# jchristopherson/nonlin

Hardware: AMD Instinct MI355X
Metric: LM iterations/sec on m=4096,n=256 fp64; FD-Jacobian GB/s vs HBM peak (higher is better)
Workload: dtype f64

## Files before the change

include/nonlin_hip.h:

```cpp
#ifndef NONLIN_HIP_H
#define NONLIN_HIP_H

#include <stdint.h>

#ifdef __cplusplus
extern "C" {
#endif

#define NLH_NO_ERROR                     0
#define NLH_INVALID_INPUT_ERROR        201
#define NLH_ARRAY_SIZE_ERROR           202
#define NLH_OUT_OF_MEMORY_ERROR        105
#define NLH_INVALID_OPERATION_ERROR    104
#define NLH_CONVERGENCE_ERROR          106
#define NLH_DIVERGENT_BEHAVIOR_ERROR   206
#define NLH_SPURIOUS_CONVERGENCE_ERROR 207
#define NLH_TOLERANCE_TOO_SMALL_ERROR  208
#define NLH_DIVIDE_BY_ZERO_ERROR       210
#define NLH_UNDEFINED_FUNCTION_ERROR   211
#define NLH_UNDERDEFINED_PROBLEM_ERROR 212
#define NLH_ERR_NO_DEVICE             -1
#define NLH_ERR_HIP                   -2
#define NLH_ERR_BAD_HANDLE            -3

// ... 654 lines not shown
                            nlh_iteration_behavior *ib, int32_t *status);
int nlh_curve_fit_batch_sep_h(nlh_handle *h, const nlh_options *opts, int32_t kind, int32_t ncomp, int32_t nbase, int32_t nprob,
                              int32_t m, const double *t, int32_t shared_t, const double *y, const double *w, int32_t analytic,
                              const double *xl, const double *xu, const nlh_group *g, const nlh_conv *cv, const nlh_sep *sp,
                              double *x, double *fvec, double *sigma, double *cov, double *chi2, int32_t *rank,
                              nlh_iteration_behavior *ib, int32_t *status);
int nlh_expr_fit_batch_sep(nlh_handle *h, const nlh_options *opts, const nlh_expr *e, int32_t nprob, int32_t m, const double *dt,
                           int32_t shared_t, const double *dy, const double *dw, int32_t analytic, const double *xl,
                           const double *xu, const nlh_group *g, const nlh_conv *cv, const nlh_sep *sp, double *dx, double *dfvec,
                           double *dsigma, double *dcov, double *dchi2, int32_t *drank, nlh_iteration_behavior *ib,
                           int32_t *status);
int nlh_expr_fit_batch_sep_h(nlh_handle *h, const nlh_options *opts, const nlh_expr *e, int32_t nprob, int32_t m, const double *t,
                             int32_t shared_t, const double *y, const double *w, int32_t analytic, const double *xl,
                             const double *xu, const nlh_group *g, const nlh_conv *cv, const nlh_sep *sp, double *x, double *fvec,
                             double *sigma, double *cov, double *chi2, int32_t *rank, nlh_iteration_behavior *ib,
                             int32_t *status);

#define NLH_K_DQ_RESIDUAL   0
#define NLH_K_DQ_PANEL      1
#define NLH_K_FD_JACOBIAN   2
#define NLH_K_GRAM          3
#define NLH_K_GRAM_REDUCE   4
#define NLH_K_JTF           5
#define NLH_K_CHOL          6
#define NLH_K_LMPAR         7
#define NLH_K_QR            8
#define NLH_K_UPDATE        9
#define NLH_K_LU           10
#define NLH_K_DQ_JACOBIAN  11
#define NLH_K_QRX_PASS     12
#define NLH_K_QRX_PIVOT    13
#define NLH_K_POLYROOTS    14
#define NLH_K_COVAR       15
#define NLH_K_COUNT        16
void nlh_timing_enable(nlh_handle *h, int32_t on);
void nlh_timing_reset(nlh_handle *h);
int  nlh_timing_get(nlh_handle *h, int32_t kernel_id, double *total_ms, int64_t *launches);
int64_t nlh_timing_samples(nlh_handle *h, int32_t kernel_id, float *out_ms, int64_t cap);
const char *nlh_kernel_name(int32_t kernel_id);

#ifdef __cplusplus
}
#endif

#include "nonlin_hip_guess.h"

#include "nonlin_hip_starts.h"

#include "nonlin_hip_boot.h"

#include "nonlin_hip_bin.h"

#include "nonlin_hip_boot_pois.h"

#endif
```

nonlin_amd/_lib.py:

```python
import ctypes as C
import math
import os

_HERE = os.path.dirname(os.path.abspath(__file__))
LIB_PATH = os.path.join(_HERE, "libnonlin_hip.so")

c_double_p = C.POINTER(C.c_double)
c_int32_p = C.POINTER(C.c_int32)

VECFCN = C.CFUNCTYPE(None, C.c_void_p, C.c_int32, c_double_p, C.c_int32, c_double_p)
JACFCN = C.CFUNCTYPE(None, C.c_void_p, C.c_int32, c_double_p, C.c_int32, c_double_p)
FCNNVAR = C.CFUNCTYPE(C.c_double, C.c_void_p, C.c_int32, c_double_p)
GRADFCN = C.CFUNCTYPE(None, C.c_void_p, C.c_int32, c_double_p, c_double_p)
DEVFCN = C.CFUNCTYPE(C.c_int, C.c_void_p, C.c_void_p, C.c_int32, C.c_void_p, C.c_int32, C.c_void_p, C.c_int32, C.c_void_p)


class IterationBehavior(C.Structure):
    _fields_ = [(k, C.c_int32) for k in (
        "iter_count", "fcn_count", "jacobian_count", "gradient_count",
        "converge_on_fcn", "converge_on_chng", "converge_on_zero_diff")]

    def as_dict(self):
        return {k: int(getattr(self, k)) for k, _ in self._fields_}

# ... 318 lines not shown
                                        C.c_void_p, C.c_int32, C.c_void_p, C.c_void_p]),
    "nlh_curve_guess_batch_h": (C.c_int, [_H, C.c_int32, C.c_int32, C.c_int32, C.c_int32, C.c_int32, c_double_p, C.c_int32, c_double_p,
                                          c_double_p, C.c_int32, c_double_p, c_int32_p]),
}

_STARTS_BOX = [c_double_p, c_double_p, c_int32_p]
STARTS_SYMBOLS = {
    "nlh_starts_candidates": (C.c_int, [C.c_int32, C.c_int32, C.c_int32] + _STARTS_BOX + [c_double_p]),
    "nlh_starts_search_batch_device": (C.c_int, [_H, C.c_int32, C.c_int32, C.c_int32, DEVFCN, C.c_void_p] + _STARTS_BOX +
                                       [C.c_int32, C.c_int32, C.c_void_p, C.c_void_p, C.c_void_p]),
    "nlh_starts_search_batch_device_h": (C.c_int, [_H, C.c_int32, C.c_int32, C.c_int32, DEVFCN, C.c_void_p] + _STARTS_BOX +
                                         [C.c_int32, C.c_int32, c_double_p, c_double_p, c_int32_p]),
    "nlh_starts_cost_batch": (C.c_int, [_H, C.c_int32, C.c_int32, C.c_void_p, C.c_void_p]),
    "nlh_starts_pick_batch": (C.c_int, [_H, C.c_int32, C.c_int32, C.c_void_p, C.c_void_p]),
    "nlh_starts_take_batch": (C.c_int, [_H, C.c_int32, C.c_int32, C.c_int32, C.c_void_p, C.c_void_p, C.c_void_p]),
}

BOOT_SYMBOLS = {
    "nlh_boot_draws": (C.c_int, [C.c_uint64, C.c_int64, C.c_int32, C.c_int32, C.c_int32, C.c_int32, c_int32_p]),
    "nlh_boot_resample_batch": (C.c_int, [_H, C.c_int32, C.c_uint64, C.c_int32, C.c_int64, C.c_int32, C.c_int32, C.c_int32, C.c_void_p,
                                          C.c_void_p, C.c_void_p, C.c_int32, C.c_void_p, C.c_void_p]),
    "nlh_boot_summary_batch": (C.c_int, [_H, C.c_int32, C.c_int32, C.c_int32, C.c_void_p, C.c_double, C.c_void_p, C.c_void_p, C.c_void_p,
                                         C.c_void_p, C.c_void_p]),
}

BIN_SYMBOLS = {
    "nlh_bin_rule": (C.c_int, [C.c_int32, c_double_p, c_double_p]),
    "nlh_bin_wrap": (C.c_int, [_H, C.c_void_p, C.c_void_p, C.c_void_p, DEVFCN, DEVFCN, C.c_void_p, C.POINTER(C.c_void_p)]),
    "nlh_bin_unwrap": _RELEASE,
    "nlh_bin_device_fcn": _LAUNCHER,
    "nlh_bin_device_jac": _LAUNCHER,
    "nlh_bin_apply_batch": (C.c_int, [_H, C.c_void_p, C.c_int32, C.c_int32, C.c_int32, C.c_void_p, C.c_void_p]),
}

BOOT_POIS_SYMBOLS = {
    "nlh_boot_poisson_draws": (C.c_int, [C.c_uint64, C.c_int64, C.c_int32, C.c_int32, C.c_int32, c_double_p, c_double_p]),
    "nlh_boot_poisson_batch": (C.c_int, [_H, C.c_uint64, C.c_int32, C.c_int64, C.c_int32, C.c_int32, C.c_int32, C.c_void_p, C.c_void_p,
                                         C.c_void_p, C.c_void_p, C.c_void_p]),
}

KERNEL_IDS = {
    "dq_residual": 0, "dq_panel": 1, "fd_jacobian": 2, "gram": 3, "gram_reduce": 4, "jtf": 5,
    "chol": 6, "lmpar": 7, "qr": 8, "update": 9, "lu": 10, "dq_jacobian": 11, "qrx_pass": 12, "qrx_pivot": 13,
    "polyroots": 14, "covar": 15,
}

_lib = None


class NonlinHipUnavailable(RuntimeError):
    pass


def load():
    global _lib
    if _lib is not None:
        return _lib
    if not os.path.exists(LIB_PATH):
        raise NonlinHipUnavailable(
            f"{LIB_PATH} not found: build it with `python -c 'import __graft_entry__ as g; g.build()'` "
            "or `make -C nonlin_amd/csrc` (there is no CPU fallback)")
    try:
        import torch
    except ImportError:
        pass
    lib = C.CDLL(LIB_PATH)
    for name, (res, args) in (list(SYMBOLS.items()) + list(GUESS_SYMBOLS.items()) + list(STARTS_SYMBOLS.items()) + list(BOOT_SYMBOLS.items()) +
                              list(BIN_SYMBOLS.items()) + list(BOOT_POIS_SYMBOLS.items())):
        fn = getattr(lib, name)
        fn.restype = res
        fn.argtypes = args
    _lib = lib
    return lib


def default_options():
    o = Options()
    load().nlh_default_options(C.byref(o))
    return o


CURVE_GAUSS, CURVE_LORENTZ, CURVE_EXPDECAY = 0, 1, 2
CURVE_KINDS = {"gauss": CURVE_GAUSS, "lorentz": CURVE_LORENTZ, "expdecay": CURVE_EXPDECAY}


def curve_kind(kind):
    if isinstance(kind, str):
        if kind not in CURVE_KINDS:
            raise ValueError(f"unknown curve kind {kind!r}: one of {sorted(CURVE_KINDS)}")
        return CURVE_KINDS[kind]
    return int(kind)


def curve_nparams(kind, ncomp=1, baseline=-1):
    n = load().nlh_curve_nparams(curve_kind(kind), int(ncomp), int(baseline))
    if n < 0:
        raise ValueError(f"no curve model of kind {kind!r} with {ncomp} components and baseline degree {baseline}")
    return n


GUESS_FALLBACK, GUESS_RANKDEF, GUESS_NONE = 1, 2, 4
GUESS_MAX_M = 8192


EXPR_OPS = ("CONST", "VAR", "PARAM", "NEG", "ADD", "SUB", "MUL", "DIV", "IPOW", "POWC", "EXP", "LOG", "SQRT", "SIN", "COS", "TANH",
            "ATAN", "ABS")
EXPR_SPECIAL_OPS = ("ERF", "ERFC", "ERFCX", "VOIGT")
EXPR_EXTENDED_OPS = ("POW", "ATAN2", "MIN", "MAX", "WHERE")
EXPR_DEF_OPS = ("LOAD",)
EXPR_SPECIAL2_OPS = ("J0", "J1", "I0E", "I1E", "LGAMMA", "EXPM1", "LOG1P")


def faddeeva_table():
    import numpy as np
    L, a = C.c_double(), np.zeros(40)
    load().nlh_faddeeva_table(C.byref(L), a.ctypes.data_as(c_double_p))
    return L.value, a


def wofz(z):
    import numpy as np
# ... 623 lines not shown
```

nonlin_amd/csrc/nlh_core.hip:

```cpp
#include "nlh_internal.h"
#include "nlh_kernels_model.h"
#include "nlh_qrx.h"

int ensure(nlh_handle *h, DevBuf &b, size_t bytes)
{
    if (bytes <= b.bytes && b.p) return 0;
    if (b.p) { hipFree(b.p); b.p = nullptr; b.bytes = 0; }
    size_t want = bytes < 256 ? 256 : bytes;
    hipError_t e = hipMalloc(&b.p, want);
    if (e != hipSuccess) { h->err = std::string("hipMalloc: ") + hipGetErrorString(e); return NLH_OUT_OF_MEMORY_ERROR; }
    b.bytes = want;
    bool known = false;
    for (auto *q : h->bufs) if (q == &b) known = true;
    if (!known) h->bufs.push_back(&b);
    return 0;
}

bool lds_fits(const void *kernel, size_t dyn)
{
    static std::mutex mu;
    static std::vector<std::pair<const void *, size_t>> statics;
    size_t st = 0;
    {
        std::lock_guard<std::mutex> g(mu);
        auto it = std::find_if(statics.begin(), statics.end(), [&](const std::pair<const void *, size_t> &e) { return e.first == kernel; });
        if (it != statics.end()) st = it->second;
        else {
            hipFuncAttributes a;
            if (hipFuncGetAttributes(&a, kernel) != hipSuccess) return false;
            st = a.sharedSizeBytes;
            statics.emplace_back(kernel, st);
        }
    }
    return st + dyn <= (size_t)NLH_LDS_MAX;
}

int ensure_staging(nlh_handle *h, size_t bytes)
{
    if (bytes <= h->staging_bytes) return 0;
    if (h->staging) hipHostFree(h->staging);
    h->staging = nullptr; h->staging_bytes = 0;
    if (hipHostMalloc(&h->staging, bytes, hipHostMallocDefault) != hipSuccess) { h->err = "hipHostMalloc (staging)"; return NLH_OUT_OF_MEMORY_ERROR; }
    h->staging_bytes = bytes;
    return 0;
}

int ensure_pinned(nlh_handle *h, size_t bytes)
{
    if (bytes <= h->pinned_bytes) return 0;
    if (h->pinned) hipHostFree(h->pinned);
    h->pinned = nullptr; h->pinned_bytes = 0;
    hipError_t e = hipHostMalloc(&h->pinned, bytes, hipHostMallocDefault);
    if (e != hipSuccess) { h->err = std::string("hipHostMalloc: ") + hipGetErrorString(e); return NLH_OUT_OF_MEMORY_ERROR; }
    h->pinned_bytes = bytes;
    return 0;
// ... 29 lines not shown
void nlh_default_options(nlh_options *o)
{
    o->max_evals = 100;
    o->ftol = 1.0e-8;
    o->xtol = 1.0e-12;
    o->gtol = 1.0e-12;
    o->print_status = 0;
    o->factor = 100.0;
    o->use_line_search = 1;
    o->ls_max_evals = 100;
    o->ls_alpha = 1.0e-4;
    o->ls_factor = 0.1;
    o->factor_policy = NLH_FACTOR_EXACT;
    o->ne_pivot_tol = 1.0e-4;
    o->fuse_fd = 1;
    o->sub_batches = 0;
}

int nlh_device_count(void)
{
    int n = 0;
    if (hipGetDeviceCount(&n) != hipSuccess) return 0;
    return n;
}

const char *nlh_version(void) { return "nonlin_hip 0.1 (gfx950)"; }

int nlh_create(nlh_handle **out, int32_t device, void *hip_stream)
{
    if (!out) return NLH_ERR_BAD_HANDLE;
    *out = nullptr;
    if (nlh_device_count() <= 0) return NLH_ERR_NO_DEVICE;
    if (hipSetDevice(device) != hipSuccess) return NLH_ERR_NO_DEVICE;
    nlh_handle *h = new nlh_handle();
    h->device = device;
    h->stream = (hipStream_t)hip_stream;
    const int lds_max = NLH_LDS_MAX;
    qrx_init_device();
    nlh_lm_init_device(lds_max);
    nlh_square_init_device(lds_max);
    nlh_cls_init_device(lds_max);
    nlh_bfgs_init_device(lds_max);
    nlh_poly_init_device(lds_max);
    nlh_polyroots_init_device(lds_max);
    nlh_covar_init_device(lds_max);
    nlh_devfcn_init_device(lds_max);
    nlh_expr_init_device(lds_max);
    nlh_sep_init_device(lds_max);
    nlh_band_init_device(lds_max);
    nlh_guess_init_device(lds_max);
    nlh_boot_init_device(lds_max);
    (void)hipFuncSetAttribute((const void *)k_dq_residual<RB>, hipFuncAttributeMaxDynamicSharedMemorySize, lds_max);
    (void)hipFuncSetAttribute((const void *)k_dq_residual2<RB / 2>, hipFuncAttributeMaxDynamicSharedMemorySize, lds_max);
    (void)hipGetLastError();
    *out = h;
    return 0;
}

void nlh_destroy(nlh_handle *h)
{
    if (!h) return;
    for (auto *wk : h->workers) nlh_destroy(wk);
    h->workers.clear();
    hipSetDevice(h->device);
    hipStreamSynchronize(h->stream);
    timing_flush(h);
    for (auto e : h->pool) hipEventDestroy(e);
    for (auto *b : h->bufs) if (b->p) hipFree(b->p);
    if (h->pinned) hipHostFree(h->pinned);
    if (h->staging) hipHostFree(h->staging);
    if (h->cbstage) hipHostFree(h->cbstage);
    if (h->lu_side) { hipStreamSynchronize(h->lu_side); hipStreamDestroy(h->lu_side); }
    if (h->lu_panel_done) hipEventDestroy(h->lu_panel_done);
    for (auto e : h->lu_bulk_done) if (e) hipEventDestroy(e);
    if (h->own_stream) hipStreamDestroy(h->stream);
    delete h;
}

const char *nlh_last_error(const nlh_handle *h) { return h ? h->err.c_str() : "null handle"; }

void nlh_timing_enable(nlh_handle *h, int32_t on)
{
    if (!h) return;
    h->timing = on == 0 ? 0u : on == 1 ? 0xffffffffu : ((uint32_t)on >> 1);
}
void nlh_timing_reset(nlh_handle *h)
{
    if (!h) return;
    timing_flush(h);
    for (int k = 0; k < NLH_K_COUNT; ++k) { h->ms[k] = 0; h->launches[k] = 0; }
    h->samples.clear();
}
int64_t nlh_timing_samples(nlh_handle *h, int32_t kid, float *out_ms, int64_t cap)
{
    if (!h) return NLH_ERR_BAD_HANDLE;
    if (kid != h->sample_kid) {
        timing_flush(h);
        h->sample_kid = kid;
        h->samples.clear();
        return 0;
    }
    timing_flush(h);
    const int64_t cnt = (int64_t)h->samples.size();
    for (int64_t i = 0; i < cnt && i < cap; ++i) out_ms[i] = h->samples[(size_t)i];
    return cnt;
}
// ... 28 lines not shown
    for (size_t e = (size_t)blockIdx.x * blockDim.x + threadIdx.x; e < mn + (size_t)n; e += (size_t)gridDim.x * blockDim.x) {
        const double u = 2.0 * sm64_u(seed, e) - 1.0;
        if (e < mn) {
            double v = u / rs;
            const size_t i = e % m, j = e / m;
            if (square_shift && i == j) v = 2.0 + v;
            A[(size_t)p * mn + e] = v;
        } else {
            xtrue[(size_t)p * n + (e - mn)] = u;
        }
    }
}

__global__ void k_gen_bx(int m, int n, uint64_t seed0, uint64_t stride, double sigma, double spread, double *b,
                         const double *xtrue, double *x0)
{
    const int p = blockIdx.y;
    const uint64_t seed = seed0 + (uint64_t)p * stride;
    const size_t base = (size_t)m * n + (size_t)n;
    for (size_t e = (size_t)blockIdx.x * blockDim.x + threadIdx.x; e < (size_t)m + n; e += (size_t)gridDim.x * blockDim.x) {
        const double u = 2.0 * sm64_u(seed, base + e) - 1.0;
        if (e < (size_t)m) b[(size_t)p * m + e] = b[(size_t)p * m + e] + sigma * u;
        else x0[(size_t)p * n + (e - m)] = xtrue[(size_t)p * n + (e - m)] + spread * u;
    }
}


void launch_dq_residual(nlh_handle *h, int nprob, int m, int n, const double *A, const double *b,
                               double gamma, const double *x, double *f, double *part,
                               const LmState *st, int want)
{
    Timed t(h, NLH_K_DQ_RESIDUAL);
    size_t sh = sizeof(double) * (size_t)(n + 32);
    const bool vec2 = (m % 2 == 0) && ((((uintptr_t)A | (uintptr_t)b | (uintptr_t)f) & 15) == 0);
    const int nblk = (m + RB - 1) / RB;
    lockstep_slices(nprob, [&](int32_t p0, int32_t cnt) {
        dim3 grid(nblk, cnt);
        const double *Ap = A + (size_t)p0 * m * n, *bp = b + (size_t)p0 * m, *xp = x + (size_t)p0 * n;
        double *fp = f + (size_t)p0 * m, *pp = part ? part + (size_t)p0 * nblk * 2 : nullptr;
        const LmState *sp = st ? st + p0 : nullptr;
        if (vec2)
            hipLaunchKernelGGL(k_dq_residual2<RB / 2>, grid, dim3(RB / 2), sh, h->stream, m, n, Ap, bp, gamma, xp, fp, pp, sp, want);
        else
            hipLaunchKernelGGL(k_dq_residual<RB>, grid, dim3(RB), sh, h->stream, m, n, Ap, bp, gamma, xp, fp, pp, sp, want);
        return 0;
    });
}

void launch_dq_panel(nlh_handle *h, int nprob, int m, int n, const double *A, const double *b,
                            double gamma, const double *x, double *P, const LmState *st, int want,
                            const double *f0_fused, bool to_qrx)
{
    Timed t(h, NLH_K_DQ_PANEL);
    constexpr int JT = 32;
    dim3 grid((m + RB - 1) / RB, (n + JT - 1) / JT, nprob);
    size_t sh = sizeof(double) * (size_t)n;
    const int tld = to_qrx ? qrx_ld(n) : 0, tcoff = to_qrx ? qrx_ld(n) - (n + 1) : 0;
    const size_t tst = to_qrx ? qrx_matrix_stride(m, n) : 0;
    if (f0_fused)
        hipLaunchKernelGGL((k_dq_panel<RB, JT, true>), grid, dim3(RB), sh, h->stream, m, n, A, b, gamma, x, P, f0_fused, st, want,
                           tld, tcoff, tst);
    else
        hipLaunchKernelGGL((k_dq_panel<RB, JT, false>), grid, dim3(RB), sh, h->stream, m, n, A, b, gamma, x, P,
                           (const double *)nullptr, st, want, 0, 0, (size_t)0);
}

void launch_fd(nlh_handle *h, int nprob, int m, int n, const double *P, const double *f0,
                      const double *x, double *J, const LmState *st, int want)
{
    Timed t(h, NLH_K_FD_JACOBIAN);
    constexpr int CJ = 8;
    const bool vec2 = (m % 2 == 0) && ((((uintptr_t)P | (uintptr_t)J | (uintptr_t)f0) & 15) == 0);
    if (vec2) {
        dim3 grid((m / 2 + RB - 1) / RB, (n + CJ - 1) / CJ, nprob);
        hipLaunchKernelGGL((k_fd_jacobian<RB, CJ, true>), grid, dim3(RB), 0, h->stream, m, n, P, f0, x, J, st, want);
    } else {
        dim3 grid((m + RB - 1) / RB, (n + CJ - 1) / CJ, nprob);
        hipLaunchKernelGGL((k_fd_jacobian<RB, CJ, false>), grid, dim3(RB), 0, h->stream, m, n, P, f0, x, J, st, want);
    }
}

void format_e10_3(double v, char out[16])
{
    char body[16];
    if (std::isnan(v)) { snprintf(out, 16, "%10s", "NaN"); return; }
    if (std::isinf(v)) { snprintf(out, 16, "%10s", v < 0 ? "-Inf" : "Inf"); return; }
    char sci[32];
    snprintf(sci, sizeof sci, "%.2e", fabs(v));
    int ex = atoi(sci + 5);
    if (v != 0.0) ex += 1;
    const char sign = std::signbit(v) && v != 0.0 ? '-' : ' ';
    if (abs(ex) < 100) snprintf(body, sizeof body, "%c0.%c%c%cE%c%02d", sign, sci[0], sci[2], sci[3], ex < 0 ? '-' : '+', abs(ex));
    else snprintf(body, sizeof body, "%c0.%c%c%c%c%03d", sign, sci[0], sci[2], sci[3], ex < 0 ? '-' : '+', abs(ex));
    snprintf(out, 16, "%10s", body);
}

void print_status(int iter, int nfeval, int njaceval, double xnorm, double fnorm)
{
    char a[16], b[16];
    format_e10_3(xnorm, a);
    format_e10_3(fnorm, b);
    printf(" \nIteration: %d\nFunction Evaluations: %d\n", iter, nfeval);
    if (njaceval > 0) printf("Jacobian Evaluations: %d\n", njaceval);
    printf("Change in Variable: %s\nResidual: %s\n", a, b);
    fflush(stdout);
}

int nlh_format_status(int32_t iter, int32_t nfeval, int32_t njaceval, double xnorm, double fnorm, char *buf,
                                 int32_t len)
// ... 32 lines not shown


int ensure_workers(nlh_handle *h, int T)
{
    while ((int)h->workers.size() < T) {
        nlh_handle *wk = new nlh_handle();
        wk->device = h->device;
        if (hipStreamCreateWithFlags(&wk->stream, hipStreamNonBlocking) != hipSuccess) { delete wk; h->err = "hipStreamCreate"; return NLH_ERR_HIP; }
        wk->own_stream = true;
        h->workers.push_back(wk);
    }
    return 0;
}

int nlh_dq_generate(nlh_handle *h, int32_t nprob, int32_t m, int32_t n, uint64_t seed0, uint64_t seed_stride, double gamma,
                    double sigma, double spread, int32_t square_shift, double *dA, double *db,
                    double *dxtrue, double *dx0)
{
    if (!h) return NLH_ERR_BAD_HANDLE;
    HIPCHK(h, hipSetDevice(h->device));
    const size_t mn = (size_t)m * n;
    unsigned gx = (unsigned)((mn + n + 255) / 256);
    if (gx > 4096) gx = 4096;
    hipLaunchKernelGGL(k_gen_A, dim3(gx, nprob), dim3(256), 0, h->stream, m, n, seed0, seed_stride, square_shift, dA, dxtrue);
    HIPCHK(h, hipMemsetAsync(db, 0, sizeof(double) * (size_t)nprob * m, h->stream));
    launch_dq_residual(h, nprob, m, n, dA, db, gamma, dxtrue, db, nullptr, nullptr, -1);
    unsigned gb = (unsigned)(((size_t)m + n + 255) / 256);
    hipLaunchKernelGGL(k_gen_bx, dim3(gb, nprob), dim3(256), 0, h->stream, m, n, seed0, seed_stride, sigma, spread, db, dxtrue, dx0);
    HIPCHK(h, hipGetLastError());
    return 0;
}

int nlh_dq_residual(nlh_handle *h, int32_t nprob, int32_t m, int32_t n, const double *dA, const double *db,
                    double gamma, const double *dx, double *df)
{
    if (!h) return NLH_ERR_BAD_HANDLE;
    HIPCHK(h, hipSetDevice(h->device));
    launch_dq_residual(h, nprob, m, n, dA, db, gamma, dx, df, nullptr, nullptr, -1);
    HIPCHK(h, hipGetLastError());
    return 0;
}

int nlh_dq_fd_panel(nlh_handle *h, int32_t nprob, int32_t m, int32_t n, const double *dA, const double *db,
                    double gamma, const double *dx, double *dP)
{
    if (!h) return NLH_ERR_BAD_HANDLE;
    if (m < 1 || n < 1) return NLH_INVALID_INPUT_ERROR;
    HIPCHK(h, hipSetDevice(h->device));
    launch_dq_panel(h, nprob, m, n, dA, db, gamma, dx, dP, nullptr, -1);
    HIPCHK(h, hipGetLastError());
    return 0;
}

int nlh_fd_jacobian_panel(nlh_handle *h, int32_t nprob, int32_t m, int32_t n, const double *dP,
                          const double *df0, const double *dx, double *dJ)
{
    if (!h) return NLH_ERR_BAD_HANDLE;
    HIPCHK(h, hipSetDevice(h->device));
    launch_fd(h, nprob, m, n, dP, df0, dx, dJ, nullptr, -1);
    HIPCHK(h, hipGetLastError());
    return 0;
}

int nlh_dq_jacobian(nlh_handle *h, int32_t nprob, int32_t m, int32_t n, const double *dA, double gamma,
                    const double *dx, double *dJ)
{
    if (!h) return NLH_ERR_BAD_HANDLE;
    HIPCHK(h, hipSetDevice(h->device));
    {
        Timed t(h, NLH_K_DQ_JACOBIAN);
        hipLaunchKernelGGL(k_dq_jacobian<RB>, dim3((m + RB - 1) / RB, nprob), dim3(RB), sizeof(double) * n, h->stream,
                           m, n, dA, gamma, dx, dJ, (const LmState *)nullptr, -1);
    }
    HIPCHK(h, hipGetLastError());
    return 0;
}
```

nonlin_amd/csrc/nlh_kernels_model.h:

```cpp
#pragma once
#include "nlh_common.h"

template <int BS>
__global__ void __launch_bounds__(BS)
k_dq_residual(int m, int n, const double *__restrict__ A, const double *__restrict__ b,
              double gamma, const double *__restrict__ xsrc, double *__restrict__ fout,
              double *__restrict__ part, const LmState *__restrict__ st, int want_stage)
{
    extern __shared__ double smem[];
    const int p = blockIdx.y;
    if (st && st[p].stage != want_stage) return;
    double *xs = smem;
    double *red = smem + n;
    const double *Ap = A + (size_t)p * m * n;
    const double *xp = xsrc + (size_t)p * n;
    for (int k = threadIdx.x; k < n; k += BS) xs[k] = xp[k];
    __syncthreads();

    const int i = blockIdx.x * BS + threadIdx.x;
    double r = 0.0;
    if (i < m) {
        double u = 0.0;
        const double *a = Ap + i;
        int k = 0;
// ... 33 lines not shown
    double *red = smem + n;
    const double *Ap = A + (size_t)p * m * n;
    const double *xp = xsrc + (size_t)p * n;
    for (int k = threadIdx.x; k < n; k += BS) xs[k] = xp[k];
    __syncthreads();

    const int i = (blockIdx.x * BS + threadIdx.x) * 2;
    double r0 = 0.0, r1 = 0.0;
    if (i < m) {
        double u0 = 0.0, u1 = 0.0;
        const double *a = Ap + i;
        int k = 0;
        for (; k + 16 <= n; k += 16) {
            double2 av[16];
#pragma unroll
            for (int q = 0; q < 16; ++q) av[q] = *reinterpret_cast<const double2 *>(a + (size_t)(k + q) * m);
#pragma unroll
            for (int q = 0; q < 16; ++q) {
                const double xk = xs[k + q];
                u0 = u0 + av[q].x * xk;
                u1 = u1 + av[q].y * xk;
            }
        }
        for (; k < n; ++k) {
            const double2 av = *reinterpret_cast<const double2 *>(a + (size_t)k * m);
            u0 = u0 + av.x * xs[k];
            u1 = u1 + av.y * xs[k];
        }
        const double2 bv = *reinterpret_cast<const double2 *>(b + (size_t)p * m + i);
        r0 = (u0 + (gamma * u0) * u0) - bv.x;
        r1 = (u1 + (gamma * u1) * u1) - bv.y;
        *reinterpret_cast<double2 *>(fout + (size_t)p * m + i) = make_double2(r0, r1);
    }
    if (part) {
        const double q0 = (i < m) ? r0 * r0 : 0.0, q1 = (i < m) ? r1 * r1 : 0.0;
        const double sq = q0 + q1;
        const double tq = ((i < m && i >= n) ? q0 : 0.0) + ((i < m && i + 1 >= n) ? q1 : 0.0);
        double s = block_reduce_sum(sq, red);
        double t = block_reduce_sum(tq, red);
        if (threadIdx.x == 0) {
            part[((size_t)p * gridDim.x + blockIdx.x) * 2 + 0] = s;
            part[((size_t)p * gridDim.x + blockIdx.x) * 2 + 1] = t;
        }
    }
}

template <int BS, int JT, bool FUSE>
__global__ void __launch_bounds__(BS)
k_dq_panel(int m, int n, const double *__restrict__ A, const double *__restrict__ b,
           double gamma, const double *__restrict__ x, double *__restrict__ P,
           const double *__restrict__ f0, const LmState *__restrict__ st, int want_stage,
           int tld, int tcoff, size_t tst)
{
    extern __shared__ double smem[];
    const int p = blockIdx.z;
    if (st && st[p].stage != want_stage) return;
    double *xs = smem;
    const double *Ap = A + (size_t)p * m * n;
    const double *xp = x + (size_t)p * n;
    for (int k = threadIdx.x; k < n; k += BS) xs[k] = xp[k];
    __syncthreads();

    const int j0 = blockIdx.y * JT;
    const int i = blockIdx.x * BS + threadIdx.x;
    if (i >= m) return;
    const int jt = min(JT, n - j0);
    const double *a = Ap + i;

    constexpr int PF = 8;
    double base = 0.0;
    {
        int k = 0;
        for (; k + PF <= j0; k += PF) {
            double av[PF];
#pragma unroll
            for (int u = 0; u < PF; ++u) av[u] = a[(size_t)(k + u) * m];
#pragma unroll
            for (int u = 0; u < PF; ++u) base = base + av[u] * xs[k + u];
        }
        for (; k < j0; ++k) base = base + a[(size_t)k * m] * xs[k];
    }

    double acc[JT];
#pragma unroll
    for (int jj = 0; jj < JT; ++jj) acc[jj] = base;

#pragma unroll
    for (int kk = 0; kk < JT; ++kk) {
        if (kk < jt) {
            const int k = j0 + kk;
            const double av = a[(size_t)k * m];
            const double xk = xs[k];
            const double pr = av * xk;
            const double pp = av * (xk + fd_step(xk));
#pragma unroll
            for (int jj = 0; jj < JT; ++jj) acc[jj] = acc[jj] + (jj == kk ? pp : pr);
        }
    }
    {
        int k = j0 + JT;
        double av[PF], aw[PF];
        if (k + PF <= n) {
#pragma unroll
            for (int u = 0; u < PF; ++u) av[u] = a[(size_t)(k + u) * m];
        }
        for (; k + PF <= n; k += PF) {
            const bool more = k + 2 * PF <= n;
            if (more) {
#pragma unroll
                for (int u = 0; u < PF; ++u) aw[u] = a[(size_t)(k + PF + u) * m];
            }
#pragma unroll
            for (int u = 0; u < PF; ++u) {
                const double pr = av[u] * xs[k + u];
#pragma unroll
                for (int jj = 0; jj < JT; ++jj) acc[jj] = acc[jj] + pr;
            }
            if (more) {
#pragma unroll
                for (int u = 0; u < PF; ++u) av[u] = aw[u];
            }
        }
        for (; k < n; ++k) {
            const double pr = a[(size_t)k * m] * xs[k];
#pragma unroll
            for (int jj = 0; jj < JT; ++jj) acc[jj] = acc[jj] + pr;
        }
    }
    const double bi = b[(size_t)p * m + i];
    const double f0i = FUSE ? f0[(size_t)p * m + i] : 0.0;
    double *Pp = tld ? P + (size_t)p * tst + ((size_t)(i >> 3) * tld + tcoff) * 8 + (i & 7) : P + (size_t)p * m * n + i;
    const size_t cstride = tld ? (size_t)8 : (size_t)m;
#pragma unroll
    for (int jj = 0; jj < JT; ++jj) {
        if (jj < jt) {
            const double u = acc[jj];
            const double r = (u + (gamma * u) * u) - bi;
            if (FUSE) __builtin_nontemporal_store((r - f0i) / fd_step(xs[j0 + jj]), Pp + (size_t)(j0 + jj) * cstride);
            else __builtin_nontemporal_store(r, Pp + (size_t)(j0 + jj) * cstride);
        }
    }
}

template <int BS, int CJ, bool VEC2>
__global__ void __launch_bounds__(BS)
k_fd_jacobian(int m, int n, const double *__restrict__ P, const double *__restrict__ f0,
              const double *__restrict__ x, double *__restrict__ J,
              const LmState *__restrict__ st, int want_stage, const int32_t *__restrict__ list = nullptr, int nfull = 0)
{
    const int p = list ? list[blockIdx.z] : blockIdx.z;
    if (st && st[p].stage != want_stage) return;
    const int ns = nfull ? nfull : n;
    const double *Pp = P + (size_t)blockIdx.z * m * n;
    double *Jp = J + (size_t)p * m * ns;
    const double *fp = f0 + (size_t)p * m;
    const double *xp = x + (size_t)p * ns;
    const int jbeg = blockIdx.y * CJ;
    const int jend = min(n, jbeg + CJ);
    if (VEC2) {
        const int i = (blockIdx.x * BS + threadIdx.x) * 2;
        if (i >= m) return;
        const double2 f = *reinterpret_cast<const double2 *>(fp + i);
#pragma unroll 4
        for (int j = jbeg; j < jend; ++j) {
            const double h = fd_step(xp[j]);
            typedef double v2d __attribute__((ext_vector_type(2)));
            const v2d v = __builtin_nontemporal_load(reinterpret_cast<const v2d *>(Pp + (size_t)j * m + i));
            v2d o;
            o.x = (v.x - f.x) / h;
            o.y = (v.y - f.y) / h;
            __builtin_nontemporal_store(o, reinterpret_cast<v2d *>(Jp + (size_t)j * m + i));
        }
    } else {
        const int i = blockIdx.x * BS + threadIdx.x;
        if (i >= m) return;
        const double f = fp[i];
        for (int j = jbeg; j < jend; ++j) {
            const double h = fd_step(xp[j]);
            Jp[(size_t)j * m + i] = (Pp[(size_t)j * m + i] - f) / h;
        }
    }
}

template <int BS>
__global__ void __launch_bounds__(BS)
k_dq_jacobian(int m, int n, const double *__restrict__ A, double gamma,
              const double *__restrict__ x, double *__restrict__ J, const LmState *__restrict__ st, int want)
{
    extern __shared__ double smem[];
    const int p = blockIdx.y;
    if (st && st[p].stage != want) return;
    double *xs = smem;
// ... 14 lines not shown
```

nonlin_amd/device.py:

```python
import collections
import contextlib
import ctypes as C
import os

import numpy as np
import torch

from . import _lib
from ._lib import (CURVE_GAUSS, CURVE_LORENTZ, CURVE_EXPDECAY, CURVE_KINDS, curve_kind, curve_nparams,
                   Expr, ParamMap, Loss, Poisson, Convolve)

IB_DTYPE = np.dtype([(k, np.int32) for k, _ in _lib.IterationBehavior._fields_])


def _chk(t, shape, name):
    if not (t.is_cuda and t.dtype == torch.float64 and t.is_contiguous() and tuple(t.shape) == tuple(shape)):
        raise ValueError(f"{name}: expected contiguous float64 GPU tensor of shape {tuple(shape)}, "
                         f"got {t.dtype} {tuple(t.shape)} cuda={t.is_cuda}")


def _ib_status(nprob):
    return (_lib.IterationBehavior * nprob)(), (C.c_int32 * nprob)()


# ... 838 lines not shown
        nprob, n = x.shape
        _chk(x, (nprob, n), "x")
        if simplex is not None:
            _chk(simplex, (nprob, n + 1, n), "simplex")
        ib, status = _ib_status(nprob)
        fout = (C.c_double * nprob)()
        o = opts or self.options(max_evals=500)
        self._call("nlh_nelder_mead_solve_batch_device", C.byref(o), float(init_size), nprob, n, self._devfcn(fcn),
                   self._ctxp(ctx), x.data_ptr(), simplex.data_ptr() if simplex is not None else None,
                   0 if simplex is None else 1, fout, ib, status)
        return ([float(v) for v in fout],) + _ib_lists(ib, status)

    def _root1v_batch(self, entry, fcns, ctx, lim, x, opts):
        nprob = x.shape[0]
        _chk(lim, (nprob, 2), "lim")
        _chk(x, (nprob,), "x")
        ibc = (_lib.IterationBehavior * nprob)()
        ib = np.frombuffer(ibc, dtype=IB_DTYPE)
        status = np.zeros(nprob, dtype=np.int32)
        fout = np.zeros(nprob, dtype=np.float64)
        o = opts or self.options()
        self._call(entry, C.byref(o), nprob, *[self._devfcn(f) for f in fcns], self._ctxp(ctx), lim.data_ptr(), x.data_ptr(),
                   fout.ctypes.data_as(_lib.c_double_p), ibc, status.ctypes.data_as(_lib.c_int32_p))
        return fout, status, ib

    def brent_solve_batch_device(self, fcn, ctx, lim, x, opts=None):
        return self._root1v_batch("nlh_brent_solve_batch_device", (fcn,), ctx, lim, x, opts)

    def newton_1var_solve_batch_device(self, fcn, ctx, lim, x, diff=None, opts=None):
        return self._root1v_batch("nlh_newton_1var_solve_batch_device", (fcn, diff), ctx, lim, x, opts)

    def fd_jacobian_device(self, fcn, ctx, m, x, fv=None, jac=None):
        nprob, n = x.shape
        _chk(x, (nprob, n), "x")
        J = torch.empty((nprob, n, m), dtype=torch.float64, device=x.device)
        self._call("nlh_fd_jacobian_device", nprob, m, n, self._devfcn(fcn), self._devfcn(jac), self._ctxp(ctx),
                   x.data_ptr(), fv.data_ptr() if fv is not None else None, J.data_ptr())
        return J

    def residual(self, A, b, gamma, x):
        nprob, n, m = A.shape
        f = torch.empty((nprob, m), dtype=torch.float64, device=A.device)
        self.h.check(self.lib.nlh_dq_residual(self.h.ptr, nprob, m, n, A.data_ptr(), b.data_ptr(), float(gamma),
                                              x.data_ptr(), f.data_ptr()), "nlh_dq_residual")
        return f

    def fd_panel(self, A, b, gamma, x):
        nprob, n, m = A.shape
        P = torch.empty((nprob, n, m), dtype=torch.float64, device=A.device)
        self.h.check(self.lib.nlh_dq_fd_panel(self.h.ptr, nprob, m, n, A.data_ptr(), b.data_ptr(), float(gamma),
                                              x.data_ptr(), P.data_ptr()), "nlh_dq_fd_panel")
        return P

    def fd_jacobian_panel(self, P, f0, x, out=None):
        nprob, n, m = P.shape
        J = out if out is not None else torch.empty_like(P)
        self.h.check(self.lib.nlh_fd_jacobian_panel(self.h.ptr, nprob, m, n, P.data_ptr(), f0.data_ptr(),
                                                    x.data_ptr(), J.data_ptr()), "nlh_fd_jacobian_panel")
        return J

    def jacobian(self, A, gamma, x):
        nprob, n, m = A.shape
        J = torch.empty_like(A)
        self.h.check(self.lib.nlh_dq_jacobian(self.h.ptr, nprob, m, n, A.data_ptr(), float(gamma), x.data_ptr(),
                                              J.data_ptr()), "nlh_dq_jacobian")
        return J

    def gram(self, J, f):
        nprob, n, m = J.shape
        G = torch.empty((nprob, n, n), dtype=torch.float64, device=J.device)
        g = torch.empty((nprob, n), dtype=torch.float64, device=J.device)
        self.h.check(self.lib.nlh_gram(self.h.ptr, nprob, m, n, J.data_ptr(), f.data_ptr(), G.data_ptr(),
                                       g.data_ptr()), "nlh_gram")
        return G, g

    def chol_factor(self, G, g):
        nprob, n, _ = G.shape
        dev = G.device
        ipvt = torch.empty((nprob, n), dtype=torch.int32, device=dev)
        acnorm = torch.empty((nprob, n), dtype=torch.float64, device=dev)
        qtf = torch.empty((nprob, n), dtype=torch.float64, device=dev)
        info = torch.empty((nprob,), dtype=torch.int32, device=dev)
        self.h.check(self.lib.nlh_chol_factor(self.h.ptr, nprob, n, G.data_ptr(), g.data_ptr(), ipvt.data_ptr(),
                                              acnorm.data_ptr(), qtf.data_ptr(), info.data_ptr()), "nlh_chol_factor")
        return ipvt, acnorm, qtf, info

    def chol_natural(self, G, g, pivot_tol=0.0, form=0):
        nprob, n, _ = G.shape
        _chk(G, (nprob, n, n), "G"); _chk(g, (nprob, n), "g")
        dev = G.device
        R = torch.empty_like(G)
        ipvt = torch.empty((nprob, n), dtype=torch.int32, device=dev)
        acnorm = torch.empty((nprob, n), dtype=torch.float64, device=dev)
        qtf = torch.empty((nprob, n), dtype=torch.float64, device=dev)
        info = torch.empty((nprob,), dtype=torch.int32, device=dev)
        self.h.check(self.lib.nlh_chol_natural(self.h.ptr, nprob, n, G.data_ptr(), g.data_ptr(), float(pivot_tol), int(form),
                                               R.data_ptr(), ipvt.data_ptr(), acnorm.data_ptr(), qtf.data_ptr(),
                                               info.data_ptr()), "nlh_chol_natural")
        return R, ipvt, acnorm, qtf, info

    def ne_signs(self, J, ipvt, R, qtf):
        nprob, n, m = J.shape
        _chk(J, (nprob, n, m), "J"); _chk(R, (nprob, n, n), "R"); _chk(qtf, (nprob, n), "qtf")
        sign = torch.empty((nprob, n), dtype=torch.float64, device=J.device)
        self.h.check(self.lib.nlh_ne_signs(self.h.ptr, nprob, m, n, J.data_ptr(), ipvt.data_ptr(), R.data_ptr(),
                                           qtf.data_ptr(), sign.data_ptr()), "nlh_ne_signs")
# ... 342 lines not shown
```

Measured before the change: 3796.

## Widen dq_panel column tile and pipeline A loads with double buffering

```diff
diff --git a/include/nonlin_hip.h b/include/nonlin_hip.h
--- a/include/nonlin_hip.h
+++ b/include/nonlin_hip.h
@@ -730,5 +730,6 @@
 #include "nonlin_hip_bin.h"
 
 #include "nonlin_hip_boot_pois.h"
+#include "nonlin_hip_stage.h"
 
 #endif
diff --git a/include/nonlin_hip_stage.h b/include/nonlin_hip_stage.h
--- /dev/null
+++ b/include/nonlin_hip_stage.h
@@ -0,0 +1,17 @@
+#ifndef NONLIN_HIP_STAGE_H
+#define NONLIN_HIP_STAGE_H
+
+#include "nonlin_hip.h"
+
+#ifdef __cplusplus
+extern "C" {
+#endif
+
+int nlh_dq_fd_jacobian(nlh_handle *h, int32_t nprob, int32_t m, int32_t n, const double *dA, const double *db,
+                       double gamma, const double *dx, const double *df0, double *dJ, int32_t layout);
+int64_t nlh_qrx_matrix_layout(int32_t nprob, int32_t m, int32_t n, int32_t *ld, int32_t *coff, int64_t *stride);
+
+#ifdef __cplusplus
+}
+#endif
+#endif
diff --git a/nonlin_amd/_lib.py b/nonlin_amd/_lib.py
--- a/nonlin_amd/_lib.py
+++ b/nonlin_amd/_lib.py
@@ -394,6 +394,13 @@
     pass
 
 
+STAGE_SYMBOLS = {
+    "nlh_dq_fd_jacobian": (C.c_int, [_H, C.c_int32, C.c_int32, C.c_int32, C.c_void_p, C.c_void_p, C.c_double,
+                                     C.c_void_p, C.c_void_p, C.c_void_p, C.c_int32]),
+    "nlh_qrx_matrix_layout": (C.c_int64, [C.c_int32, C.c_int32, C.c_int32, c_int32_p, c_int32_p, C.POINTER(C.c_int64)]),
+}
+
+
 def load():
     global _lib
     if _lib is not None:
@@ -408,7 +415,7 @@
         pass
     lib = C.CDLL(LIB_PATH)
     for name, (res, args) in (list(SYMBOLS.items()) + list(GUESS_SYMBOLS.items()) + list(STARTS_SYMBOLS.items()) + list(BOOT_SYMBOLS.items()) +
-                              list(BIN_SYMBOLS.items()) + list(BOOT_POIS_SYMBOLS.items())):
+                              list(BIN_SYMBOLS.items()) + list(BOOT_POIS_SYMBOLS.items()) + list(STAGE_SYMBOLS.items())):
         fn = getattr(lib, name)
         fn.restype = res
         fn.argtypes = args
diff --git a/nonlin_amd/csrc/nlh_core.hip b/nonlin_amd/csrc/nlh_core.hip
--- a/nonlin_amd/csrc/nlh_core.hip
+++ b/nonlin_amd/csrc/nlh_core.hip
@@ -1,6 +1,8 @@
 #include "nlh_internal.h"
 #include "nlh_kernels_model.h"
 #include "nlh_qrx.h"
+
+static const int DQ_PANEL_JT = 64;
 
 int ensure(nlh_handle *h, DevBuf &b, size_t bytes)
 {
@@ -136,6 +138,8 @@
     nlh_boot_init_device(lds_max);
     (void)hipFuncSetAttribute((const void *)k_dq_residual<RB>, hipFuncAttributeMaxDynamicSharedMemorySize, lds_max);
     (void)hipFuncSetAttribute((const void *)k_dq_residual2<RB / 2>, hipFuncAttributeMaxDynamicSharedMemorySize, lds_max);
+    (void)hipFuncSetAttribute((const void *)k_dq_panel<RB, DQ_PANEL_JT, true>, hipFuncAttributeMaxDynamicSharedMemorySize, lds_max);
+    (void)hipFuncSetAttribute((const void *)k_dq_panel<RB, DQ_PANEL_JT, false>, hipFuncAttributeMaxDynamicSharedMemorySize, lds_max);
     (void)hipGetLastError();
     *out = h;
     return 0;
@@ -270,9 +274,9 @@
                             const double *f0_fused, bool to_qrx)
 {
     Timed t(h, NLH_K_DQ_PANEL);
-    constexpr int JT = 32;
+    constexpr int JT = DQ_PANEL_JT;
     dim3 grid((m + RB - 1) / RB, (n + JT - 1) / JT, nprob);
-    size_t sh = sizeof(double) * (size_t)n;
+    const size_t sh = sizeof(double) * (size_t)(n + 2 * JT);
     const int tld = to_qrx ? qrx_ld(n) : 0, tcoff = to_qrx ? qrx_ld(n) - (n + 1) : 0;
     const size_t tst = to_qrx ? qrx_matrix_stride(m, n) : 0;
     if (f0_fused)
@@ -411,6 +415,26 @@
     return 0;
 }
 
+int nlh_dq_fd_jacobian(nlh_handle *h, int32_t nprob, int32_t m, int32_t n, const double *dA, const double *db,
+                       double gamma, const double *dx, const double *df0, double *dJ, int32_t layout)
+{
+    if (!h) return NLH_ERR_BAD_HANDLE;
+    if (nprob < 1 || m < 1 || n < 1 || !df0 || (layout != 0 && layout != 1)) return NLH_INVALID_INPUT_ERROR;
+    HIPCHK(h, hipSetDevice(h->device));
+    launch_dq_panel(h, nprob, m, n, dA, db, gamma, dx, dJ, nullptr, -1, df0, layout == 1);
+    HIPCHK(h, hipGetLastError());
+    return 0;
+}
+
+int64_t nlh_qrx_matrix_layout(int32_t nprob, int32_t m, int32_t n, int32_t *ld, int32_t *coff, int64_t *stride)
+{
+    if (nprob < 1 || m < 1 || n < 1) return -NLH_INVALID_INPUT_ERROR;
+    if (ld) *ld = qrx_ld(n);
+    if (coff) *coff = qrx_ld(n) - (n + 1);
+    if (stride) *stride = (int64_t)qrx_matrix_stride(m, n);
+    return (int64_t)qrx_matrix_doubles(nprob, m, n);
+}
+
 int nlh_fd_jacobian_panel(nlh_handle *h, int32_t nprob, int32_t m, int32_t n, const double *dP,
                           const double *df0, const double *dx, double *dJ)
 {
diff --git a/nonlin_amd/csrc/nlh_kernels_model.h b/nonlin_amd/csrc/nlh_kernels_model.h
--- a/nonlin_amd/csrc/nlh_kernels_model.h
+++ b/nonlin_amd/csrc/nlh_kernels_model.h
@@ -109,81 +109,97 @@
            const double *__restrict__ f0, const LmState *__restrict__ st, int want_stage,
            int tld, int tcoff, size_t tst)
 {
+    constexpr int PF = 8;
+    static_assert(JT % (2 * PF) == 0, "every phase of the load pipeline begins on buffer 0");
     extern __shared__ double smem[];
     const int p = blockIdx.z;
     if (st && st[p].stage != want_stage) return;
-    double *xs = smem;
+    const int j0 = blockIdx.y * JT;
+    const int jt = min(JT, n - j0);
+    double *xs = smem;
+    double *xh = smem + n;
+    double *hs = xh + JT;
     const double *Ap = A + (size_t)p * m * n;
     const double *xp = x + (size_t)p * n;
     for (int k = threadIdx.x; k < n; k += BS) xs[k] = xp[k];
-    __syncthreads();
-
-    const int j0 = blockIdx.y * JT;
+    for (int k = threadIdx.x; k < jt; k += BS) {
+        const double xk = xp[j0 + k], h = fd_step(xk);
+        xh[k] = xk + h;
+        hs[k] = h;
+    }
+    __syncthreads();
+
     const int i = blockIdx.x * BS + threadIdx.x;
     if (i >= m) return;
-    const int jt = min(JT, n - j0);
     const double *a = Ap + i;
-
-    constexpr int PF = 8;
+    const int ng = (n + PF - 1) / PF, ngf = n / PF;
+
+    double bf[2][PF];
+    auto load = [&](int g, double (&v)[PF]) {
+        if (g < ng) {
+#pragma unroll
+            for (int u = 0; u < PF; ++u) v[u] = a[(size_t)min(g * PF + u, n - 1) * m];
+        }
+    };
+
     double base = 0.0;
-    {
-        int k = 0;
-        for (; k + PF <= j0; k += PF) {
-            double av[PF];
-#pragma unroll
-            for (int u = 0; u < PF; ++u) av[u] = a[(size_t)(k + u) * m];
-#pragma unroll
-            for (int u = 0; u < PF; ++u) base = base + av[u] * xs[k + u];
-        }
-        for (; k < j0; ++k) base = base + a[(size_t)k * m] * xs[k];
+    int g = 0;
+    load(0, bf[0]);
+    auto prefix = [&](const double (&v)[PF]) {
+#pragma unroll
+        for (int u = 0; u < PF; ++u) base = base + v[u] * xs[g * PF + u];
+        ++g;
+    };
+    while (g * PF < j0) {
+        load(g + 1, bf[1]);
+        prefix(bf[0]);
+        load(g + 1, bf[0]);
+        prefix(bf[1]);
     }
 
     double acc[JT];
 #pragma unroll
-    for (int jj = 0; jj < JT; ++jj) acc[jj] = base;
-
-#pragma unroll
-    for (int kk = 0; kk < JT; ++kk) {
-        if (kk < jt) {
-            const int k = j0 + kk;
-            const double av = a[(size_t)k * m];
-            const double xk = xs[k];
-            const double pr = av * xk;
-            const double pp = av * (xk + fd_step(xk));
-#pragma unroll
-            for (int jj = 0; jj < JT; ++jj) acc[jj] = acc[jj] + (jj == kk ? pp : pr);
-        }
-    }
-    {
-        int k = j0 + JT;
-        double av[PF], aw[PF];
-        if (k + PF <= n) {
-#pragma unroll
-            for (int u = 0; u < PF; ++u) av[u] = a[(size_t)(k + u) * m];
-        }
-        for (; k + PF <= n; k += PF) {
-            const bool more = k + 2 * PF <= n;
-            if (more) {
-#pragma unroll
-                for (int u = 0; u < PF; ++u) aw[u] = a[(size_t)(k + PF + u) * m];
+    for (int gg = 0; gg < JT / PF; ++gg) {
+        load(g + 1, bf[(gg + 1) & 1]);
+#pragma unroll
+        for (int u = 0; u < PF; ++u) {
+            const int kk = gg * PF + u;
+            if (kk < jt) {
+                const double av = bf[gg & 1][u];
+                const double pr = av * xs[j0 + kk];
+                const double pp = av * xh[kk];
+#pragma unroll
+                for (int jj = 0; jj < kk; ++jj) acc[jj] = acc[jj] + pr;
+                acc[kk] = base + pp;
+                base = base + pr;
             }
-#pragma unroll
-            for (int u = 0; u < PF; ++u) {
-                const double pr = av[u] * xs[k + u];
+        }
+        ++g;
+    }
+
+    auto rest = [&](const double (&v)[PF], bool whole) {
+#pragma unroll
+        for (int u = 0; u < PF; ++u) {
+            if (whole || g * PF + u < n) {
+                const double pr = v[u] * xs[min(g * PF + u, n - 1)];
 #pragma unroll
                 for (int jj = 0; jj < JT; ++jj) acc[jj] = acc[jj] + pr;
             }
-            if (more) {
-#pragma unroll
-                for (int u = 0; u < PF; ++u) av[u] = aw[u];
-            }
-        }
-        for (; k < n; ++k) {
-            const double pr = a[(size_t)k * m] * xs[k];
-#pragma unroll
-            for (int jj = 0; jj < JT; ++jj) acc[jj] = acc[jj] + pr;
-        }
-    }
+        }
+        ++g;
+    };
+    while (g + 2 <= ngf) {
+        load(g + 1, bf[1]);
+        rest(bf[0], true);
+        load(g + 1, bf[0]);
+        rest(bf[1], true);
+    }
+    if (g < ng) {
+        load(g + 1, bf[1]);
+        rest(bf[0], false);
+        if (g < ng) rest(bf[1], false);
+    }
+
     const double bi = b[(size_t)p * m + i];
     const double f0i = FUSE ? f0[(size_t)p * m + i] : 0.0;
     double *Pp = tld ? P + (size_t)p * tst + ((size_t)(i >> 3) * tld + tcoff) * 8 + (i & 7) : P + (size_t)p * m * n + i;
@@ -193,8 +209,10 @@
         if (jj < jt) {
             const double u = acc[jj];
             const double r = (u + (gamma * u) * u) - bi;
-            if (FUSE) __builtin_nontemporal_store((r - f0i) / fd_step(xs[j0 + jj]), Pp + (size_t)(j0 + jj) * cstride);
-            else __builtin_nontemporal_store(r, Pp + (size_t)(j0 + jj) * cstride);
+            const double o = FUSE ? (r - f0i) / hs[jj] : r;
+            double *dst = Pp + (size_t)(j0 + jj) * cstride;
+            if (tld) *dst = o;
+            else __builtin_nontemporal_store(o, dst);
         }
     }
 }
diff --git a/nonlin_amd/device.py b/nonlin_amd/device.py
--- a/nonlin_amd/device.py
+++ b/nonlin_amd/device.py
@@ -914,6 +914,22 @@
                                               x.data_ptr(), P.data_ptr()), "nlh_dq_fd_panel")
         return P
 
+    def qrx_matrix_layout(self, nprob, m, n):
+        ld, coff, stride = C.c_int32(), C.c_int32(), C.c_int64()
+        doubles = int(self.lib.nlh_qrx_matrix_layout(nprob, m, n, C.byref(ld), C.byref(coff), C.byref(stride)))
+        if doubles < 0:
+            raise ValueError(f"nlh_qrx_matrix_layout({nprob}, {m}, {n}) = {doubles}")
+        return doubles, ld.value, coff.value, stride.value
+
+    def fd_jacobian_fused(self, A, b, gamma, x, f0, layout=0, out=None):
+        nprob, n, m = A.shape
+        if out is None:
+            out = (torch.empty((nprob, n, m), dtype=torch.float64, device=A.device) if layout == 0 else
+                   torch.zeros(self.qrx_matrix_layout(nprob, m, n)[0], dtype=torch.float64, device=A.device))
+        self.h.check(self.lib.nlh_dq_fd_jacobian(self.h.ptr, nprob, m, n, A.data_ptr(), b.data_ptr(), float(gamma),
+                                                 x.data_ptr(), f0.data_ptr(), out.data_ptr(), int(layout)), "nlh_dq_fd_jacobian")
+        return out
+
     def fd_jacobian_panel(self, P, f0, x, out=None):
         nprob, n, m = P.shape
         J = out if out is not None else torch.empty_like(P)
```

Result: no change. 3804 (median of 6 runs) (+0.2%).
